# pd3/bcftools

Measured on AMD Instinct MI355X. Metric: variant sites/sec (mpileup|call -m), 1000-sample 30x WGS synthetic, higher is better.
Workload: dtype u8/i32 + f64 likelihood sums

## Files before the change

### bcftools_amd/csrc/glfgen.hip

```cpp
#include <hip/hip_runtime.h>
#include <cstdlib>
#include "kernels.h"

namespace bcfgpu {

#define WG 256
#ifndef GLF_WAVES
#define GLF_WAVES 5
#endif
#define DEF_MAPQ 20
#define CAP_DIST 25

#define NT16_INT_TBL 0x4444444344424104ull
__device__ __forceinline__ int nt16_int(int c) { return (int)((NT16_INT_TBL >> (4 * (c & 15))) & 7); }
__device__ __forceinline__ int tri(int j, int k) { return k * (k + 1) / 2 + j; }

__device__ __forceinline__ uint32_t wave_sum_u32(uint32_t v)
{
    #pragma unroll
    for (int o = 32; o > 0; o >>= 1) v += __shfl_xor(v, o);
    return v;
}

#define LDS_FK   0
#define LDS_CNT  2112
#ifndef NRANK
#define NRANK 10
#endif
#define NSLOT    NRANK
#ifndef FU
#define FU       4
#endif
#define LDS_HIST_OFF (LDS_CNT + NSLOT * WG * 4)
#define HP_SIZE 280
#define HP_MQS  220
#define HP_MAX  0xffffu
static_assert(GLF_MAX_WINDOW <= HP_MAX, "one round's window alone must fit a 16-bit half of the packed histograms");
static_assert(H_SIZE <= 2 * HP_SIZE, "a deep cell's 32-bit histograms take the LDS of two packed slots (hist_slots >= 2 whenever it is not 0)");
#define NPART 17
static_assert(NPART == SITE_NSUM + 3, "phase A's partial sums: the site totals and three mapQ >= 59 counts");

#define KEY_PACK(rev, q, b, sc) ((uint32_t)(rev) | (uint32_t)(q) << 1 | (uint32_t)(b) << 7 | (uint32_t)(sc) << 10)
#define KEY_REV(k)  ((k) & 1u)
#define KEY_Q(k)    (((k) >> 1) & 63u)
#define KEY_B(k)    (((k) >> 7) & 7u)
#define KEY_SC(k)   (((k) >> 10) & 1u)
#define KEY_PRIM    0x800u

#ifndef WR
#define WR 2
#endif
struct PrimSrc {
    const uint16_t *kpp;
    __device__ __forceinline__ uint32_t key(int j) const { return kpp[j]; }
    __device__ __forceinline__ bool ok(uint32_t k) const { return k != 0; }
    __device__ __forceinline__ int operator()(int j) const { const uint32_t k = key(j); return ok(k) ? (int)(k & 0x7f) : -1; }
};
struct BaseSrc {
    const uint16_t *kp; int b;
    __device__ __forceinline__ uint32_t key(int i) const { return kp[i]; }
    __device__ __forceinline__ bool ok(uint32_t k) const { return KEY_B(k) == (uint32_t)b; }
    __device__ __forceinline__ int operator()(int i) const { const uint32_t k = key(i); return ok(k) ? (int)(k & 0x7f) : -1; }
};
__device__ __forceinline__ uint32_t popc64(uint64_t x) { return (uint32_t)__popc((uint32_t)x) + (uint32_t)__popc((uint32_t)(x >> 32)); }
template <bool FIRST, bool CHK, class Src>
__device__ __forceinline__ void count_keys(uint32_t *s_slot, uint64_t qm, int tid, Src src, int nsrc)
{
    const uint64_t qm1 = qm >> 1;
    for (int j = 0; __any(j < nsrc); j += FU) {
        if (j < nsrc) {
            uint32_t k4[FU];
            #pragma unroll
            for (int u = 0; u < FU; ++u) k4[u] = src.key(j + u);
            #pragma unroll
            for (int u = 0; u < FU; ++u) {
                const uint32_t k = k4[u], q = KEY_Q(k);
                const uint32_t r = popc64(qm1 >> q);
                bool take = src.ok(k) && (u == 0 || j + u < nsrc);
                if (!FIRST) take = take && ((qm >> q) & 1ull);
                if (CHK) take = take && r < (uint32_t)NRANK;
                const uint32_t rv = (uint32_t)((int32_t)(k << 31) >> 31);
                if (take) atomicAdd(&s_slot[r * WG + tid], (rv & 1u) | (~rv & 0x100u));
            }
        }
    }
}
template <bool FIRST, class Src>
__device__ __forceinline__ uint32_t count_runs(uint32_t *s_slot, uint64_t qm, int tid, Src src, int nsrc)
{
    #pragma unroll
    for (int k = 0; k < NRANK; ++k) s_slot[k * WG + tid] = 0;
    if (__any(popc64(qm) > (uint32_t)NRANK)) count_keys<FIRST, true>(s_slot, qm, tid, src, nsrc);
    else count_keys<FIRST, false>(s_slot, qm, tid, src, nsrc);
    uint32_t qs = 0;
    uint64_t m = qm;
    #pragma unroll
    for (int r = 0; r < NRANK && __any(m != 0); ++r) {
        if (m != 0) {
            const uint32_t q = 63u - (uint32_t)__builtin_clzll(m);
            const uint32_t c = s_slot[r * WG + tid];
            s_slot[r * WG + tid] = c | q << 16;
            qs = __builtin_amdgcn_udot4(c, q | q << 8, qs, false);
            m &= ~(1ull << q);
        }
    }
    return qs;
}

template <class Src>
__device__ __forceinline__ double walk_runs(uint32_t *s_slot, uint64_t qm, const double *s_fk, const char *bbase, int tid,
                                            uint32_t brow, Src src, int nsrc, uint32_t &rev_out, uint32_t &qs_out)
{
    double bs = 0;
    uint32_t qs = 0;
    uint32_t wpack = 0;
    uint32_t cnt = 0;
    uint32_t koff = brow;
    uint32_t qoff = 0;
    uint32_t r = 0;
    uint32_t d_nx = 0;
    auto slot_of = [&](uint32_t rk) -> uint32_t { return s_slot[min(rk, (uint32_t)NRANK - 1u) * WG + tid]; };
    auto step = [&](uint32_t (&off)[WR], uint32_t (&wi)[WR]) -> bool {
        const bool pop = cnt == 0 && r < NRANK;
        cnt = pop ? (d_nx & 0xffu) | (d_nx & 0xff00u) << 8 : cnt;
        qoff = pop ? (d_nx & 0x3f0000u) << 3 : qoff;
        r += pop ? 1u : 0u;
        d_nx = slot_of(r);
        const uint32_t sh = (cnt & 0xffffu) ? 0u : 16u;
        const uint32_t left = (cnt >> sh) & 0xffffu;
        const uint32_t w = (wpack >> sh) & 0xffffu;
        const uint32_t o1 = qoff + koff;
        #pragma unroll
        for (uint32_t u = 0; u < WR; ++u) {
            const bool act = left > u;
            wi[u] = act ? w + u : 256u;
            off[u] = act ? o1 + (u << 11) : brow;
        }
        const uint32_t took = min(left, (uint32_t)WR);
        wpack += took << sh; cnt -= took << sh;
        koff += took << 11;
        return __any(left != 0);
    };
    #define WALK_LOAD(B, F, off_, wi_) do { _Pragma("unroll") for (int u_ = 0; u_ < WR; ++u_) { \
        B[u_] = *reinterpret_cast<const double*>(bbase + (off_)[u_]); F[u_] = s_fk[(wi_)[u_]]; } } while (0)
    #define WALK_ADD(B, F) do { _Pragma("unroll") for (int u_ = 0; u_ < WR; ++u_) bs += F[u_] * B[u_]; } while (0)
    bool first = true;
    while (__any(qm != 0)) {
        qs += first ? count_runs<true>(s_slot, qm, tid, src, nsrc) : count_runs<false>(s_slot, qm, tid, src, nsrc);
        first = false; r = 0;
        d_nx = slot_of(0);
        double bx[WR], fx[WR], by[WR], fy[WR];
        uint32_t off[WR], wi[WR];
        bool ax = step(off, wi);
        WALK_LOAD(bx, fx, off, wi);
        bool ay = step(off, wi);
        WALK_LOAD(by, fy, off, wi);
        while (ax) {
            WALK_ADD(bx, fx);
            ax = step(off, wi);
            WALK_LOAD(bx, fx, off, wi);
            if (!ay) break;
            WALK_ADD(by, fy);
            ay = step(off, wi);
            WALK_LOAD(by, fy, off, wi);
        }
        WALK_ADD(bx, fx);
        WALK_ADD(by, fy);
        if (__any(__popcll(qm) > NRANK)) {
            uint64_t m = qm;
            for (int k = 0; k < NRANK && m; ++k) m &= ~(1ull << (63 - __clzll((long long)m)));
            qm = m;
        } else qm = 0;
    }
    #undef WALK_ADD
    #undef WALK_LOAD
    rev_out = wpack & 0xffffu; qs_out = qs;
    return bs;
}

struct ReadSums {
    uint32_t t_bq, t_bq2, t_mq, t_mq2, t_md, t_md2;
    uint32_t d_bq, d_bq2, d_mq, d_mq2, d_md, d_md2;
    __device__ __forceinline__ void clear() { t_bq = t_bq2 = t_mq = t_mq2 = t_md = t_md2 = d_bq = d_bq2 = d_mq = d_mq2 = d_md = d_md2 = 0; }
};
struct ReadCounts {
    uint32_t ori, mq0, m59, ref59, rev59;
    __device__ __forceinline__ void clear() { ori = mq0 = m59 = ref59 = rev59 = 0; }
};
typedef unsigned short v2u16 __attribute__((ext_vector_type(2)));

__device__ __forceinline__ uint32_t perm(uint32_t hi, uint32_t lo, uint32_t sel) { return __builtin_amdgcn_perm(hi, lo, sel); }
#define SEL_EVEN 0x0c020c00u
#define SEL_ODD  0x0c030c01u
#define SEL_JOIN 0x06020400u
#define SEL_GE8  0x07030501u
__device__ __forceinline__ v2u16 as_v2(uint32_t x) { return __builtin_bit_cast(v2u16, x); }
__device__ __forceinline__ uint32_t as_u(v2u16 x) { return __builtin_bit_cast(uint32_t, x); }
__device__ __forceinline__ uint32_t pk_min(uint32_t a, uint32_t b) { return as_u(__builtin_elementwise_min(as_v2(a), as_v2(b))); }
__device__ __forceinline__ uint32_t pk_max(uint32_t a, uint32_t b) { return as_u(__builtin_elementwise_max(as_v2(a), as_v2(b))); }
__device__ __forceinline__ uint32_t nonzero80(uint32_t x) { return (((x & 0x7f7f7f7fu) + 0x7f7f7f7fu) | x) & 0x80808080u; }
__device__ __forceinline__ uint32_t bytes_of80(uint32_t m) { return m | (m - (m >> 7)); }
__device__ __forceinline__ uint32_t byte_at(uint32_t x, int u) { return (x >> (8 * u)) & 0xffu; }

template <bool INDEL, bool LDS_HIST, bool DEEP>
__global__ __launch_bounds__(WG) __attribute__((amdgpu_waves_per_eu(GLF_WAVES, GLF_WAVES))) void glfgen_kernel(const GlfgenParams P)
{
    extern __shared__ __align__(16) unsigned char smem[];
    if (DEEP && (blockIdx.x >= P.deep_ctr[0] || P.deep_list[2 * blockIdx.x] == 0xffffffffu)) return;
    const int cap = DEEP ? 0x7ffffff0 : P.lds_cap;
    double   *s_fk  = reinterpret_cast<double*>(smem + LDS_FK);
    uint32_t *s_cnt = reinterpret_cast<uint32_t*>(smem + LDS_CNT);
    int      *s_hist = reinterpret_cast<int*>(smem + LDS_HIST_OFF);
    unsigned long long *s_tot = reinterpret_cast<unsigned long long*>(s_hist + (size_t)P.hist_slots * HP_SIZE);
    uint32_t *s_part = s_cnt;
    const int pcol = P.part_cols;
    uint16_t *s_key = DEEP ? P.deep_keys + P.deep_list[2 * blockIdx.x + 1]
                           : reinterpret_cast<uint16_t*>(s_tot + (size_t)P.hist_slots * SITE_NSUM);
    __shared__ unsigned int s_next, s_skip, s_pend;
    constexpr bool PACKED = LDS_HIST && !DEEP;

    const int tid = threadIdx.x;
    const int S = P.n_smpl;
    const long ncells = (long)P.n_sites * S;
    const long cell0 = DEEP ? (long)P.deep_list[2 * blockIdx.x] : (long)blockIdx.x * WG;
    const long cell_end = DEEP ? cell0 + 1 : min(cell0 + WG, ncells);
    const int site0 = (int)(cell0 / S);
    const int site_last = (int)((cell_end - 1) / S);

    const long cell = cell0 + tid;
    const bool active = cell < cell_end;

    s_fk[tid] = P.fk[tid];
    if (tid < 8) s_fk[256 + tid] = 0.0;
    if (LDS_HIST) {
        for (int i = tid; i < P.hist_slots * HP_SIZE; i += WG) s_hist[i] = 0;
        for (int i = tid; i < P.hist_slots * SITE_NSUM; i += WG) s_tot[i] = 0;
    }

    int site = 0, ref4c = 4;
    uint32_t beg = 0, end = 0;
    if (active) {
        site = (int)(cell / S);
        beg = P.off[cell]; end = P.off[cell + 1];
        if (!INDEL) ref4c = nt16_int(P.ref16[site]);
    }
    const int primary = INDEL ? 0 : ref4c;
    uint32_t fmt_flag = (uint32_t)P.fmt_flag;
    asm volatile("" : "+s"(fmt_flag));
    const bool want_epos = (fmt_flag & (BCFGPU_INFO_RPB | BCFGPU_INFO_VDB)) != 0;
    const bool want_scr = (fmt_flag & (BCFGPU_INFO_SCR | BCFGPU_FMT_SCR)) != 0;
    const uint32_t span_end = P.off[cell_end];
    uint32_t n_reads_tot = P.n_reads, min_baseQ = (uint32_t)P.min_baseQ, capQ = (uint32_t)P.capQ;
    asm volatile("" : "+s"(n_reads_tot), "+s"(min_baseQ), "+s"(capQ));
    const uint32_t *p_rd = P.rd, *p_aux = P.aux, *p_off = P.off;
    const uint8_t *p_epos = P.epos;
    asm volatile("" : "+s"(p_rd), "+s"(p_aux), "+s"(p_off), "+s"(p_epos));

    bool done = !active;
    bool deep = false;
    if (!DEEP && active && end - beg > (uint32_t)cap - 3u) {
        deep = true;
        const uint32_t need = (end - beg + 16u) & ~7u;
        const uint32_t slot = atomicAdd(&P.deep_ctr[0], 1u), at = atomicAdd(&P.deep_ctr[1], need);
        const bool room = at + need <= P.deep_key_cap;
        if (slot < P.deep_cap) { P.deep_list[2 * slot] = room ? (uint32_t)cell : 0xffffffffu; P.deep_list[2 * slot + 1] = room ? at : 0u; }
        if (slot >= P.deep_cap || !room) { atomicExch(P.err, BCFGPU_E_DEPTH); atomicExch(&P.deep_ctr[2], 1u); }
    }
    uint32_t base = p_off[cell0];
    if (PACKED && tid == 0) s_pend = min((base & ~3u) + (uint32_t)cap, span_end) - base;

    auto flush_packed = [&](const bool clear) {
        const int nslot = min(P.hist_slots, P.n_sites - site0);
        for (int i = tid; i < nslot * HP_SIZE; i += WG) {
            const uint32_t v = (uint32_t)s_hist[i];
            if (!v) continue;
            if (clear) s_hist[i] = 0;
            const int sl = i / HP_SIZE, j = i - sl * HP_SIZE;
            int *g = P.hist + (long)(site0 + sl) * H_SIZE;
            const int lo = j < HP_MQS ? j : H_FWD_MQS + (j - HP_MQS), hi = j < HP_MQS ? j + H_ALT_OFF : H_REV_MQS + (j - HP_MQS);
            if (v & 0xffffu) atomicAdd(&g[lo], (int)(v & 0xffffu));
            if (v >> 16) atomicAdd(&g[hi], (int)(v >> 16));
        }
    };

    for (;;) {
        const uint32_t abase = base & ~3u;
        const uint32_t lim = DEEP ? span_end : min(abase + (uint32_t)cap, span_end);
        if (tid == 0) { s_next = 0xffffffffu; s_skip = 0; }
        if (LDS_HIST) {
            int i0 = tid;
            asm volatile("" : "+v"(i0));
            for (int i = i0; i < P.hist_slots * NPART * pcol; i += WG) s_part[i] = 0;
        }
        __syncthreads();
        const bool cand = !done && !deep && beg >= base && end <= lim;
        if (!done && !cand) atomicMin(&s_next, beg);
        __syncthreads();
        const uint32_t nb = s_next;
        const uint32_t rlim = min(nb, lim);
        const bool part = cand && end <= rlim;

        for (int sg = site0; sg <= site_last; ++sg) {
            const long c_lo = max(cell0, (long)sg * S), c_hi = min(cell_end, (long)(sg + 1) * S);
            const uint32_t rb = max(p_off[c_lo], base), re = min(p_off[c_hi], rlim);
            if (rb >= re) continue;
            const int ref_base = INDEL ? -1 : (int)P.ref16[sg];
            const uint32_t ref4 = INDEL ? 4u : (uint32_t)nt16_int(ref_base);
            const uint32_t primq = INDEL ? 0u : ref4;
            const unsigned long long tbl = (NT16_INT_TBL & ~0xfull) | (unsigned long long)ref4;
            int *hist = LDS_HIST ? s_hist + (sg - site0) * HP_SIZE : P.hist + (long)sg * H_SIZE;
            ReadSums A; A.clear();
            ReadCounts C; C.clear();
            const uint32_t tlo_lo = 0x04010000u | ref4, tlo_hi = 0x04040402u, thi_lo = 0x04040403u, thi_hi = 0x04040404u;
            const uint32_t kq = 0x01000100u - min(min_baseQ, 256u) * 0x00010001u;
            const uint32_t cap2 = min(capQ, 0xffffu) * 0x00010001u;
            const uint32_t refb4 = (uint32_t)(ref_base & 15) * 0x01010101u, prim4 = primq * 0x01010101u;
            const uint32_t scm = want_scr ? 0x04040404u : 0u;
            const bool all_diff = !INDEL && ref4 >= 4;
            const bool no_ref = INDEL || ref_base < 0 || ref_base > 15;

            auto quad = [&](const uint4 &w4, const uint4 &a4, uint32_t e4, uint32_t vm4, uint32_t &k01, uint32_t &k23) {
                const uint32_t t0 = perm(w4.y, w4.x, 0x05010400u), t1 = perm(w4.y, w4.x, 0x07030602u);
                const uint32_t t2 = perm(w4.w, w4.z, 0x05010400u), t3 = perm(w4.w, w4.z, 0x07030602u);
                uint32_t B4 = perm(t2, t0, 0x05040100u);
                const uint32_t M4 = perm(t2, t0, 0x07060302u);
                const uint32_t F4 = (vm4 & perm(t3, t1, 0x05040100u)) | (~vm4 & 0x80808080u);
                const uint32_t D4 = perm(t3, t1, 0x07060302u);
                uint32_t QR4, BB4;
                uint32_t ok80;
                const uint32_t seen80 = (INDEL ? F4 : F4 | F4 << 1) & 0x80808080u ^ 0x80808080u;
                if (INDEL) {
                    uint32_t qv[4], bv[4];
                    const uint32_t av[4] = { a4.x, a4.y, a4.z, a4.w }, wv[4] = { w4.x, w4.y, w4.z, w4.w };
                    #pragma unroll
                    for (int u = 0; u < 4; ++u) {
                        const uint32_t ax = av[u];
                        uint32_t b = (ax >> 16) & 0xf, q = ax & 0xff;
                        if (q < min_baseQ) { b = 0; q = wv[u] & 0xff; }
                        bv[u] = min(b, 4u);
                        qv[u] = min(q, (ax >> 8) & 0xff);
                    }
                    B4 = perm(perm(a4.w, a4.z, 0x04000c0cu), perm(a4.y, a4.x, 0x0c0c0400u), 0x07060100u);
                    QR4 = qv[0] | qv[1] << 8 | qv[2] << 16 | qv[3] << 24;
                    BB4 = bv[0] | bv[1] << 8 | bv[2] << 16 | bv[3] << 24;
                    ok80 = seen80;
                } else {
                    const uint32_t ge = perm(perm(0, B4, SEL_ODD) + kq, perm(0, B4, SEL_EVEN) + kq, SEL_GE8);
                    ok80 = seen80 & ge << 7;
                    QR4 = B4;
                    const uint32_t s = F4 & 0x07070707u;
                    BB4 = perm(perm(thi_hi, thi_lo, s), perm(tlo_hi, tlo_lo, s), 0x03020100u | (F4 >> 1 & 0x04040404u));
                }
                const uint32_t OK4 = bytes_of80(ok80);
                const uint32_t me = perm(0, M4, SEL_EVEN), mo = perm(0, M4, SEL_ODD);
                const uint32_t mfe = pk_min(me + (uint32_t)__mul24((int)perm(0, me + 0x00010001u, SEL_ODD), DEF_MAPQ - 255), cap2);
                const uint32_t mfo = pk_min(mo + (uint32_t)__mul24((int)perm(0, mo + 0x00010001u, SEL_ODD), DEF_MAPQ - 255), cap2);
                const uint32_t qe = pk_max(pk_min(pk_min(perm(0, QR4, SEL_EVEN), mfe), 0x003f003fu), 0x00040004u);
                const uint32_t qo = pk_max(pk_min(pk_min(perm(0, QR4, SEL_ODD), mfo), 0x003f003fu), 0x00040004u);
                const uint32_t Q4 = perm(qo, qe, SEL_JOIN);
                const uint32_t Mf4 = perm(mfo, mfe, SEL_JOIN);
                const uint32_t Df4 = perm(pk_min(perm(0, D4, SEL_ODD), 0x00190019u), pk_min(perm(0, D4, SEL_EVEN), 0x00190019u), SEL_JOIN);
                const uint32_t m59_80 = ok80 & perm(mfo + 0x00c500c5u, mfe + 0x00c500c5u, SEL_GE8) << 7;
                const uint32_t nref80 = no_ref ? 0x80808080u : nonzero80((F4 ^ refb4) & 0x0f0f0f0fu);
                C.ori += __builtin_popcount(seen80);
                C.mq0 += __builtin_popcount(ok80 & ~nonzero80(M4));
                C.m59 += __builtin_popcount(m59_80);
                C.ref59 += __builtin_popcount(m59_80 & ~nref80);
                C.rev59 += __builtin_popcount(m59_80 & F4 << 3);
                const uint32_t nprim80 = nonzero80(BB4 ^ prim4);
                const uint32_t klo = (((F4 >> 4) & 0x01010101u) | Q4 << 1 | (BB4 & 0x01010101u) << 7) & OK4;
                const uint32_t khi = (((BB4 >> 1) & 0x03030303u) | ((F4 >> 3) & scm) | ((nprim80 ^ 0x80808080u) >> 4)) & OK4;
                k01 = perm(khi, klo, 0x05010400u); k23 = perm(khi, klo, 0x07030602u);
                const uint32_t Bm = B4 & OK4, Mm = Mf4 & OK4, Dm = Df4 & OK4;
                A.t_bq = __builtin_amdgcn_udot4(Bm, 0x01010101u, A.t_bq, false); A.t_bq2 = __builtin_amdgcn_udot4(Bm, Bm, A.t_bq2, false);
                A.t_mq = __builtin_amdgcn_udot4(Mm, 0x01010101u, A.t_mq, false); A.t_mq2 = __builtin_amdgcn_udot4(Mm, Mm, A.t_mq2, false);
                A.t_md = __builtin_amdgcn_udot4(Dm, 0x01010101u, A.t_md, false); A.t_md2 = __builtin_amdgcn_udot4(Dm, Dm, A.t_md2, false);
                const uint32_t dif80 = ok80 & (all_diff ? 0x80808080u : nprim80);
                if (dif80) {
                    const uint32_t DM = bytes_of80(dif80);
                    const uint32_t bd = Bm & DM, qd = Mm & DM, dd = Dm & DM;
                    A.d_bq = __builtin_amdgcn_udot4(bd, 0x01010101u, A.d_bq, false); A.d_bq2 = __builtin_amdgcn_udot4(bd, bd, A.d_bq2, false);
                    A.d_mq = __builtin_amdgcn_udot4(qd, 0x01010101u, A.d_mq, false); A.d_mq2 = __builtin_amdgcn_udot4(qd, qd, A.d_mq2, false);
                    A.d_md = __builtin_amdgcn_udot4(dd, 0x01010101u, A.d_md, false); A.d_md2 = __builtin_amdgcn_udot4(dd, dd, A.d_md2, false);
                }
                #pragma unroll
                for (int u = 0; u < 4; ++u) {
                    if (!((ok80 >> (8 * u + 7)) & 1)) continue;
                    const bool isref = !((nref80 >> (8 * u + 7)) & 1), rev = (F4 >> (8 * u + 4)) & 1;
                    const uint32_t bq = byte_at(B4, u), mapQ = byte_at(Mf4, u), pos = byte_at(e4, u);
                    const bool m59 = (m59_80 >> (8 * u + 7)) & 1;
                    if (PACKED) {
                        const int inc = isref ? 1 : 0x10000;
                        atomicAdd(&hist[H_REF_POS + pos], inc);
                        atomicAdd(&hist[H_REF_BQ + min(bq, 59u)], inc);
                        if (!m59) {
                            atomicAdd(&hist[H_REF_MQ + mapQ], inc);
                            atomicAdd(&hist[HP_MQS + mapQ], rev ? 0x10000 : 1);
                        }
                    } else {
                        const uint32_t aoff = isref ? 0u : (uint32_t)H_ALT_OFF;
                        atomicAdd(&hist[aoff + H_REF_POS + pos], 1);
                        atomicAdd(&hist[aoff + H_REF_BQ + min(bq, 59u)], 1);
                        if (!m59) {
                            atomicAdd(&hist[aoff + H_REF_MQ + mapQ], 1);
                            atomicAdd(&hist[(rev ? H_REV_MQS : H_FWD_MQS) + mapQ], 1);
                        }
                    }
                }
            };

            const uint32_t g0 = rb & ~3u;
            uint4 w4n = make_uint4(0, 0, 0, 0), a4n = make_uint4(0, 0, 0, 0);
            uint32_t e4n = 0;
            auto fetch = [&](uint32_t i4) {
                if (i4 >= re) return;
                if (i4 + 3 < n_reads_tot) {
                    w4n = *reinterpret_cast<const uint4*>(p_rd + i4);
                    if (want_epos) e4n = *reinterpret_cast<const uint32_t*>(p_epos + i4);
                    if (INDEL) a4n = *reinterpret_cast<const uint4*>(p_aux + i4);
                } else {
                    uint32_t t4[4] = {0, 0, 0, 0}, x4[4] = {0, 0, 0, 0};
                    e4n = 0;
                    for (int j = 0; j < 4; ++j) if (i4 + j < n_reads_tot) {
                        t4[j] = p_rd[i4 + j];
                        if (want_epos) e4n |= (uint32_t)p_epos[i4 + j] << (8 * j);
                        if (INDEL) x4[j] = p_aux[i4 + j];
                    }
                    w4n = make_uint4(t4[0], t4[1], t4[2], t4[3]); a4n = make_uint4(x4[0], x4[1], x4[2], x4[3]);
                }
            };
            fetch(g0 + 4u * tid);
            for (uint32_t i4 = g0 + 4u * tid; i4 < re; i4 += 4u * WG) {
                const uint4 w4 = w4n, a4 = a4n;
                const uint32_t e4 = e4n;
                fetch(i4 + 4u * WG);
                const uint32_t lo = rb > i4 ? rb - i4 : 0u, hi = min(re - i4, 4u);
                const uint32_t vm4 = (0xffffffffu << (8 * lo)) & (hi == 4u ? 0xffffffffu : ~(0xffffffffu << (8 * hi)));
                uint32_t k01, k23;
                quad(w4, a4, e4, vm4, k01, k23);
                const uint32_t ko = i4 - abase;
                if (vm4 == 0xffffffffu) {
                    *reinterpret_cast<uint2*>(s_key + ko) = make_uint2(k01, k23);
                } else {
                    const uint32_t kv[4] = { k01 & 0xffffu, k01 >> 16, k23 & 0xffffu, k23 >> 16 };
                    #pragma unroll
                    for (int u = 0; u < 4; ++u) if ((vm4 >> (8 * u)) & 1) s_key[ko + u] = (uint16_t)kv[u];
                }
            }
            const uint32_t v[NPART] = { A.t_bq - A.d_bq, A.t_bq2 - A.d_bq2, A.d_bq, A.d_bq2, A.t_mq - A.d_mq, A.t_mq2 - A.d_mq2, A.d_mq, A.d_mq2,
                                        A.t_md - A.d_md, A.t_md2 - A.d_md2, A.d_md, A.d_md2, C.ori, C.mq0, C.m59, C.ref59, C.rev59 };
            if (LDS_HIST) {
                uint32_t *pt = s_part + (sg - site0) * (NPART * pcol) + (tid & (pcol - 1));
                #pragma unroll
                for (int j = 0; j < NPART; ++j) atomicAdd(&pt[j * pcol], v[j]);
            } else {
                unsigned long long *tot = P.site_sums + (size_t)sg * SITE_NSUM;
                uint32_t x[NPART];
                #pragma unroll
                for (int j = 0; j < NPART; ++j) x[j] = wave_sum_u32(v[j]);
                if ((tid & 63) == 0) {
                    #pragma unroll
                    for (int j = 0; j < SITE_NSUM; ++j) if (x[j]) atomicAdd(&tot[j], (unsigned long long)x[j]);
                    const uint32_t m59 = x[SITE_NSUM], ref59 = x[SITE_NSUM + 1], rev59 = x[SITE_NSUM + 2];
                    if (ref59) atomicAdd(&hist[H_REF_MQ + 59], (int)ref59);
                    if (m59 - ref59) atomicAdd(&hist[H_ALT_MQ + 59], (int)(m59 - ref59));
                    if (m59 - rev59) atomicAdd(&hist[H_FWD_MQS + 59], (int)(m59 - rev59));
                    if (rev59) atomicAdd(&hist[H_REV_MQS + 59], (int)rev59);
                }
            }
        }
        __syncthreads();
        if (LDS_HIST) {
            const int nslot = min(P.hist_slots, P.n_sites - site0), q4 = pcol >> 2;
            for (int i = tid; i < nslot * NPART * 4; i += WG) {
                const uint32_t *pt = s_part + (i >> 2) * pcol + (i & 3) * q4;
                unsigned long long x = 0;
                for (int k = 0; k < q4; ++k) x += pt[k];
                x += __shfl_xor(x, 1); x += __shfl_xor(x, 2);
                if ((i & 3) == 0 && x) {
                    const int vi = i >> 2, sl = vi / NPART, j = vi % NPART;
                    if (j < SITE_NSUM) s_tot[sl * SITE_NSUM + j] += x;
                    else {
                        const int c = (int)(uint32_t)x;
                        int *g = P.hist + (long)(site0 + sl) * H_SIZE;
                        if (j == SITE_NSUM) { atomicAdd(&g[H_ALT_MQ + 59], c); atomicAdd(&g[H_FWD_MQS + 59], c); }
                        else if (j == SITE_NSUM + 1) { atomicAdd(&g[H_REF_MQ + 59], c); atomicAdd(&g[H_ALT_MQ + 59], -c); }
                        else { atomicAdd(&g[H_REV_MQS + 59], c); atomicAdd(&g[H_FWD_MQS + 59], -c); }
                    }
                }
            }
            __syncthreads();
        }

        uint16_t *kp_w = s_key + (part ? beg - abase : 0);
        const uint16_t *kp = kp_w;
        const int cnt_raw = part ? (int)(end - beg) : 0;
        if (__any(cnt_raw > BCFGPU_MAX_DEPTH)) {
            if (cnt_raw > BCFGPU_MAX_DEPTH) {
                uint32_t nus = 0;
                for (int i = 0; i < cnt_raw; ++i) nus += kp_w[i] != 0 ? 1u : 0u;
                const volatile unsigned long long *t = reinterpret_cast<const volatile unsigned long long*>(P.crp);
                uint64_t *qs64_p = reinterpret_cast<uint64_t*>(t[2]); uint32_t *misc_p = reinterpret_cast<uint32_t*>(t[6]);
                uint32_t mark = 0;
                if (nus > BCFGPU_MAX_DEPTH) {
                    uint32_t qs[4] = {0, 0, 0, 0}, af[4] = {0, 0, 0, 0}, ar[4] = {0, 0, 0, 0}, cn[4] = {0, 0, 0, 0}, sc = 0, acc = 0;
                    const bool all_diff = !INDEL && ref4c >= 4;
                    bool planned = false;
                    if (P.draw_bits) {
                        uint32_t nm = 0;
                        for (int i = 0; i < cnt_raw; ++i) { const uint32_t ri = beg + (uint32_t)i; nm += (kp_w[i] != 0 && ((P.draw_bits[ri >> 5] >> (ri & 31)) & 1u)) ? 1u : 0u; }
                        planned = nm == BCFGPU_MAX_DEPTH;
                    }
                    for (int i = 0; i < cnt_raw; ++i) {
                        const uint32_t k = kp_w[i];
                        if (k == 0) continue;
                        const uint32_t rev = KEY_REV(k), q = KEY_Q(k), b = KEY_B(k);
                        const uint32_t dr = ((all_diff || !(k & KEY_PRIM)) ? 2u : 0u) | rev;
                        #pragma unroll
                        for (uint32_t x = 0; x < 4; ++x) {
                            qs[x] += b == x ? q : 0u;
                            af[x] += (b == x && !rev) ? 1u : 0u; ar[x] += (b == x && rev) ? 1u : 0u;
                            cn[x] += dr == x ? 1u : 0u;
                        }
                        sc += KEY_SC(k);
                        bool stays = ++acc <= BCFGPU_MAX_DEPTH;
                        if (planned) { const uint32_t ri = beg + (uint32_t)i; stays = ((P.draw_bits[ri >> 5] >> (ri & 31)) & 1u) != 0; }
                        if (!stays) kp_w[i] = 0;
                    }
                    const uint32_t slot = atomicAdd(P.wide_ctr, 1u);
                    const uint32_t big = af[0] | af[1] | af[2] | af[3] | ar[0] | ar[1] | ar[2] | ar[3] | cn[0] | cn[1] | cn[2] | cn[3] | sc;
                    if (slot >= P.wide_cap || big > 0xffffu) atomicExch(P.err, BCFGPU_E_DEPTH);
                    else {
                        WideRec *w = reinterpret_cast<WideRec*>(t[7]) + slot;
                        #pragma unroll
                        for (int x = 0; x < 4; ++x) { w->qs[x] = qs[x]; w->ad[x] = af[x] | ar[x] << 16; }
                        w->cnt[0] = cn[0] | cn[1] << 16; w->cnt[1] = cn[2] | cn[3] << 16;
                        w->scr = sc; w->n = nus; w->cell = (uint32_t)cell; w->pad[0] = w->pad[1] = w->pad[2] = 0;
                        qs64_p[cell] = WIDE_QS_MARK | slot;
                        mark = CR_WIDE;
                    }
                    if (!planned) atomicAdd(P.trunc, 1u);
                }
                misc_p[cell] = mark;
            }
        }
        uint32_t scr = 0;
        if (want_scr) for (int i = 0; i < cnt_raw; ++i) scr += KEY_SC((uint32_t)kp[i]);
        uint64_t qmask = 0;
        uint32_t n_prim = 0;
        uint64_t qs64 = 0;
        uint64_t ad64 = 0;
        uint32_t n_b4 = 0;
        uint32_t o_rev = 0, n_other = 0;
        {
            uint32_t k_nx = kp[0];
            for (int i = 0; i < cnt_raw; ++i) {
                const uint32_t k = k_nx;
                k_nx = kp[i + 1];
                const uint32_t pb = k >> 11;
                qmask |= (uint64_t)pb << KEY_Q(k);
                n_prim += pb;
                if (k - 1u < KEY_PRIM - 1u) {
                    const uint32_t t = kp_w[n_other], rev = KEY_REV(k), q = KEY_Q(k), b = KEY_B(k);
                    kp_w[n_other] = (uint16_t)k; kp_w[i] = (uint16_t)t;
                    ++n_other; o_rev += rev;
                    if (b < 4) { qs64 += (uint64_t)q << (16 * b); ad64 += 1ull << (8 * b + 32 * rev); }
                    else ++n_b4;
                }
            }
        }
        const uint32_t n = n_prim + n_other;
        const bool dead_cell = n == 0;
        const char *bbase = reinterpret_cast<const char*>(P.beta);
        const uint32_t brow = n << 3;

        double bsum[5] = {0, 0, 0, 0, 0};
        uint32_t prim_rev = 0, qs_prim = 0;
        {
            const uint16_t *kpp = kp + n_other;
            const PrimSrc psrc{kpp};
            const double bs = walk_runs(s_cnt, qmask, s_fk, bbase, tid, brow, psrc, dead_cell ? 0 : cnt_raw - (int)n_other, prim_rev, qs_prim);
            #pragma unroll
            for (int b = 0; b < 5; ++b) if (b == primary) bsum[b] = bs;
        }
        if (primary < 4) {
            qs64 += (uint64_t)qs_prim << (16 * primary);
            ad64 += (uint64_t)(n_prim - prim_rev) << (8 * primary) | (uint64_t)prim_rev << (8 * primary + 32);
        } else n_b4 += n_prim;
        int c[5];
        #pragma unroll
        for (int b = 0; b < 4; ++b) c[b] = (int)((ad64 >> (8 * b)) & 0xff) + (int)((ad64 >> (8 * b + 32)) & 0xff);
        c[4] = (int)n_b4;
        if (__any(n_other > 0)) {
            #pragma unroll 1
            for (int b = 0; b < 5; ++b) {
                int cb = b == 0 ? c[0] : b == 1 ? c[1] : b == 2 ? c[2] : b == 3 ? c[3] : c[4];
                if (b == primary || dead_cell) cb = 0;
                if (!__any(cb > 0)) continue;
                const BaseSrc src{kp, b};
                const int no = cb > 0 ? (int)n_other : 0;
                double bs;
                if (!__any(cb > 1)) {
                    int key = -1;
                    for (int i = 0; __any(i < no); ++i) { const int k7 = i < no ? src(i) : -1; if (k7 >= 0) key = k7; }
                    const uint32_t off1 = key >= 0 ? ((uint32_t)(key >> 1) << 19) + brow : brow;
                    const double B1 = *reinterpret_cast<const double*>(bbase + off1);
                    const double F1 = key >= 0 ? s_fk[0] : s_fk[256];
                    bs = 0.;
                    bs += F1 * B1;
                } else {
                uint64_t qm = 0;
                for (int i = 0; i < no; ++i) { const int key = src(i); if (key >= 0) qm |= 1ull << (key >> 1); }
                uint32_t r_, q_;
                bs = walk_runs(s_cnt, qm, s_fk, bbase, tid, brow, src, no, r_, q_);
                }
                if (cb > 0) {
                    #pragma unroll
                    for (int bb = 0; bb < 5; ++bb) if (bb == b) bsum[bb] = bs;
                }
            }
        }
        const uint32_t n_rev = prim_rev + o_rev;

        uint32_t code = 0;
        CallretPlanes cr;
        {
            const volatile unsigned long long *t = reinterpret_cast<const volatile unsigned long long*>(P.crp);
            cr.p15 = reinterpret_cast<float*>(t[0]); cr.pa = reinterpret_cast<float*>(t[1]);
            cr.qs64 = reinterpret_cast<uint64_t*>(t[2]); cr.adf = reinterpret_cast<uint32_t*>(t[3]);
            cr.adr = reinterpret_cast<uint32_t*>(t[4]); cr.cnt4 = reinterpret_cast<uint32_t*>(t[5]);
            cr.misc = reinterpret_cast<uint32_t*>(t[6]);
        }
        if (part) {
            const int nbases = (c[0] > 0) + (c[1] > 0) + (c[2] > 0) + (c[3] > 0) + (c[4] > 0);
            if (nbases <= 1) {
                const int b = c[1] > 0 ? 1 : c[2] > 0 ? 2 : c[3] > 0 ? 3 : c[4] > 0 ? 4 : 0;
                double bsb = bsum[0];
                #pragma unroll
                for (int k = 1; k < 5; ++k) if (k == b) bsb = bsum[k];
                float A = n > 0 ? (float)((double)0.0f + bsb) : 0.0f;
                if (A < 0.0f) A = 0.0f;
                cr.pa[cell] = A;
                code = (uint32_t)b;
            } else {
                code = CR_FULL;
                float *p15c = cr.p15 + (size_t)cell * 16;
                #pragma unroll
                for (int j = 0; j < 5; ++j) {
                    float tmp1 = 0.0f; int tmp2 = 0;
                    #pragma unroll
                    for (int k = 0; k < 5; ++k) { if (k == j) continue; tmp1 = (float)((double)tmp1 + bsum[k]); tmp2 += c[k]; }
                    float v = 0.0f;
                    if (n > 0 && tmp2) v = tmp1;
                    if (v < 0.0f) v = 0.0f;
                    p15c[tri(j, j)] = v;
                    #pragma unroll
                    for (int k = j + 1; k < 5; ++k) {
                        const int cjk = c[j] + c[k];
                        float t1 = 0.0f; int t2 = 0;
                        #pragma unroll
                        for (int i = 0; i < 5; ++i) { if (i == j || i == k) continue; t1 = (float)((double)t1 + bsum[i]); t2 += c[i]; }
                        float h = 0.0f;
                        if (n > 0) {
                            const double lh = -4.343 * P.lhet[cjk << 8 | c[k]];
                            h = t2 ? (float)(lh + (double)t1) : (float)lh;
                            if (h < 0.0f) h = 0.0f;
                        }
                        p15c[tri(j, k)] = h;
                    }
                }
            }
        }
        if (part) {
            const bool all_diff = (!INDEL && ref4c >= 4);
            const uint32_t n_fwd = n - n_rev;
            const uint32_t d_rev = all_diff ? n_rev : o_rev, d_fwd = all_diff ? n_fwd : n_other - o_rev;
            const uint32_t cnt4 = (n_fwd - d_fwd) | (n_rev - d_rev) << 8 | d_fwd << 16 | d_rev << 24;
            uint32_t wm = 0;
            if (cnt_raw > BCFGPU_MAX_DEPTH) wm = *reinterpret_cast<volatile uint32_t*>(&cr.misc[cell]) & CR_WIDE;
            if (!wm) cr.qs64[cell] = qs64;
            cr.adf[cell] = (uint32_t)ad64; cr.adr[cell] = (uint32_t)(ad64 >> 32); cr.cnt4[cell] = cnt4;
            cr.misc[cell] = code | wm | (scr & 0xff) << 8;
            done = true;
        }
        if (nb == 0xffffffffu) break;
        base = nb;
        if (!DEEP && !done && deep && beg == base) s_skip = end;
        __syncthreads();
        if (!DEEP) {
            const uint32_t sk = s_skip, pend = PACKED ? s_pend : 0u;
            if (sk) { if (deep && beg == base) done = true; base = sk; }
            __syncthreads();
            if (PACKED) {
                const uint32_t win = min((base & ~3u) + (uint32_t)cap, span_end) - base, p = pend + win;
                const bool fl = p > HP_MAX;
                if (tid == 0) s_pend = fl ? win : p;
                if (fl) flush_packed(true);
            }
        }
    }

    if (LDS_HIST) {
        __syncthreads();
        const int nslot = min(P.hist_slots, P.n_sites - site0);
        if (PACKED) flush_packed(false);
        else {
            int *g = P.hist + (long)site0 * H_SIZE;
            for (int i = tid; i < H_SIZE; i += WG) { const int v = s_hist[i]; if (v) atomicAdd(&g[i], v); }
        }
        for (int i = tid; i < nslot * SITE_NSUM; i += WG) {
            const unsigned long long v = s_tot[i];
            if (v) atomicAdd(&P.site_sums[(size_t)site0 * SITE_NSUM + i], v);
        }
    }
}

size_t glfgen_lds_bytes(int cap, int hist_slots)
{
    return LDS_HIST_OFF + (size_t)hist_slots * (HP_SIZE * sizeof(int) + SITE_NSUM * 8) + ((size_t)cap + 8) * 2;
}

template <bool INDEL, bool LDS_HIST>
static void launch_one(const GlfgenParams &p, hipStream_t s, int grid, size_t lds)
{
    if (lds > 48 * 1024)
        hipFuncSetAttribute(reinterpret_cast<const void*>(glfgen_kernel<INDEL, LDS_HIST, false>),
                            hipFuncAttributeMaxDynamicSharedMemorySize, (int)lds);
    hipLaunchKernelGGL((glfgen_kernel<INDEL, LDS_HIST, false>), dim3(grid), dim3(WG), lds, s, p);
    if (p.deep_cap) hipLaunchKernelGGL((glfgen_kernel<INDEL, LDS_HIST, true>), dim3(p.deep_cap), dim3(WG), glfgen_lds_bytes(0, p.hist_slots), s, p);
}

void launch_glfgen(const GlfgenParams &p, hipStream_t s)
{
    const long ncells = (long)p.n_sites * p.n_smpl;
    if (ncells == 0) return;
    const int grid = (int)((ncells + WG - 1) / WG);
    const size_t lds = glfgen_lds_bytes(p.lds_cap, p.hist_slots);
    if (p.is_indel) { if (p.hist_slots) launch_one<true, true>(p, s, grid, lds); else launch_one<true, false>(p, s, grid, lds); }
    else            { if (p.hist_slots) launch_one<false, true>(p, s, grid, lds); else launch_one<false, false>(p, s, grid, lds); }
}

}
```

Measured before the change: 6.336 million.

## Sort cells by read depth within workgroup to balance wave work

Before processing, each workgroup counting-sorts its 256 cells by descending read depth, using an LDS histogram and a DPP wave prefix scan, then remaps each thread to a permuted cell. The aim is to put cells of similar depth in the same wavefront, cutting divergence and idle lanes in the per-read loops. It adds several barriers and LDS traffic at kernel start. It also changes thread-to-cell mapping, which could hurt coalescing of per-cell loads and any code that assumes tid order.

```diff
diff --git a/bcftools_amd/csrc/glfgen.hip b/bcftools_amd/csrc/glfgen.hip
--- a/bcftools_amd/csrc/glfgen.hip
+++ b/bcftools_amd/csrc/glfgen.hip
@@ -19,6 +19,16 @@
 {
     #pragma unroll
     for (int o = 32; o > 0; o >>= 1) v += __shfl_xor(v, o);
+    return v;
+}
+__device__ __forceinline__ uint32_t wave_scan_u32(uint32_t v)
+{
+    v += (uint32_t)__builtin_amdgcn_update_dpp(0, (int)v, 0x111, 0xf, 0xf, true);
+    v += (uint32_t)__builtin_amdgcn_update_dpp(0, (int)v, 0x112, 0xf, 0xf, true);
+    v += (uint32_t)__builtin_amdgcn_update_dpp(0, (int)v, 0x114, 0xf, 0xf, true);
+    v += (uint32_t)__builtin_amdgcn_update_dpp(0, (int)v, 0x118, 0xf, 0xf, true);
+    v += (uint32_t)__builtin_amdgcn_update_dpp(0, (int)v, 0x142, 0xa, 0xf, false);
+    v += (uint32_t)__builtin_amdgcn_update_dpp(0, (int)v, 0x143, 0xc, 0xf, false);
     return v;
 }
 
@@ -227,24 +237,6 @@
     const int site0 = (int)(cell0 / S);
     const int site_last = (int)((cell_end - 1) / S);
 
-    const long cell = cell0 + tid;
-    const bool active = cell < cell_end;
-
-    s_fk[tid] = P.fk[tid];
-    if (tid < 8) s_fk[256 + tid] = 0.0;
-    if (LDS_HIST) {
-        for (int i = tid; i < P.hist_slots * HP_SIZE; i += WG) s_hist[i] = 0;
-        for (int i = tid; i < P.hist_slots * SITE_NSUM; i += WG) s_tot[i] = 0;
-    }
-
-    int site = 0, ref4c = 4;
-    uint32_t beg = 0, end = 0;
-    if (active) {
-        site = (int)(cell / S);
-        beg = P.off[cell]; end = P.off[cell + 1];
-        if (!INDEL) ref4c = nt16_int(P.ref16[site]);
-    }
-    const int primary = INDEL ? 0 : ref4c;
     uint32_t fmt_flag = (uint32_t)P.fmt_flag;
     asm volatile("" : "+s"(fmt_flag));
     const bool want_epos = (fmt_flag & (BCFGPU_INFO_RPB | BCFGPU_INFO_VDB)) != 0;
@@ -256,6 +248,48 @@
     const uint8_t *p_epos = P.epos;
     asm volatile("" : "+s"(p_rd), "+s"(p_aux), "+s"(p_off), "+s"(p_epos));
 
+    uint32_t own = (uint32_t)tid;
+    if (!DEEP) {
+        uint32_t *s_bin = s_cnt, *s_wsum = s_cnt + WG;
+        uint8_t *s_perm = reinterpret_cast<uint8_t*>(s_cnt + WG + 4);
+        s_bin[tid] = 0;
+        const long c = cell0 + tid;
+        const uint32_t d = c < cell_end ? p_off[c + 1] - p_off[c] : 0u;
+        const uint32_t bin = 255u - min(d, 255u);
+        __syncthreads();
+        const uint32_t at = atomicAdd(&s_bin[bin], 1u);
+        __syncthreads();
+        const uint32_t nbin = s_bin[tid], incl = wave_scan_u32(nbin);
+        if ((tid & 63) == 63) s_wsum[tid >> 6] = incl;
+        __syncthreads();
+        uint32_t first = incl - nbin;
+        #pragma unroll
+        for (int w = 0; w < 3; ++w) first += w < (tid >> 6) ? s_wsum[w] : 0u;
+        s_bin[tid] = first;
+        __syncthreads();
+        s_perm[s_bin[bin] + at] = (uint8_t)tid;
+        __syncthreads();
+        own = s_perm[tid];
+        __syncthreads();
+    }
+    const long cell = cell0 + own;
+    const bool active = cell < cell_end;
+
+    s_fk[tid] = P.fk[tid];
+    if (tid < 8) s_fk[256 + tid] = 0.0;
+    if (LDS_HIST) {
+        for (int i = tid; i < P.hist_slots * HP_SIZE; i += WG) s_hist[i] = 0;
+        for (int i = tid; i < P.hist_slots * SITE_NSUM; i += WG) s_tot[i] = 0;
+    }
+
+    int site = 0, ref4c = 4;
+    uint32_t beg = 0, end = 0;
+    if (active) {
+        site = (int)(cell / S);
+        beg = p_off[cell]; end = p_off[cell + 1];
+        if (!INDEL) ref4c = nt16_int(P.ref16[site]);
+    }
+    const int primary = INDEL ? 0 : ref4c;
     bool done = !active;
     bool deep = false;
     if (!DEEP && active && end - beg > (uint32_t)cap - 3u) {
```

Result: no change. 6.320 million (-0.2%).
